# kelaendi/mused

Hardware: AMD Instinct MI355X
Metric: stream rows/sec, d=1024 l=128 window=10k synthetic (SWFD + kNN similarity + eigenstep + labels) (higher is better)
Workload: dtype f64; 1 GPU; synthetic d=1024 l=128 window=10000 k=50 (BASELINE config 2); stream=blob, W=10000, d=1024, l=128, k=50, modalities=1, swfd_levels=14, rccl_ranks=1, lanes_per_gpu=20, padded_window_slots=2

## Files before the change

### include/mused_hip.h

```cpp
#ifndef MUSED_HIP_H
#define MUSED_HIP_H

#ifdef __cplusplus
extern "C" {
#endif

#define MUSED_OK 0
#define MUSED_ERR_ARG -1
#define MUSED_ERR_HIP -2
#define MUSED_ERR_STATE -3
#define MUSED_ERR_UNSUPPORTED -4

#define MUSED_F32 0
#define MUSED_F64 1
#define MUSED_I64 2
#define MUSED_BITS 3

#define MUSED_METRIC_L2 0
#define MUSED_METRIC_COSINE 1

const char* mused_last_error(void);
int mused_version(void);
int mused_memcpy_d2d(void* dst, const void* src, long bytes, void* stream);

// ... 117 lines not shown
int mused_spmm_binary_path(int n, int r, long ldq, long ldy, int q_align, int y_align);
int mused_spmm_force_path(int path);
int mused_lu_permute_l(double* Y, int n, int r, long ld, int* ws_int, double* ws_f64, void* stream);
int mused_lu_mode(void);
int mused_lu_path(int n, int r);
int mused_qr_economic(double* Y, int n, int r, long ldy, double* Q, long ldq, double* ws_f64, void* stream);
int mused_syevj_batched(const double* G, int n, int batch, int sweeps, double* evals, double* V, void* stream);
int mused_gemm_f64(int a_kc, int b_kc, const double* A, long lda, const double* B, long ldb, double* C, long ldc,
                   int M, int N, int K, double alpha, void* stream);
int mused_gemm_f64_batched(int a_kc, int b_kc, const double* A, long lda, long strideA, const double* B, long ldb,
                           long strideB, double* C, long ldc, long strideC, int M, int N, int K, int batch,
                           double alpha, void* stream);
int mused_gemm_f64_batched_rep(int a_kc, int b_kc, const double* A, long lda, long strideA, const double* B, long ldb,
                               long strideB, double* C, long ldc, long strideC, int M, int N, int K, int batch,
                               double alpha, const int* rep, void* stream);
int mused_gemm_f64_splitk(int a_kc, int b_kc, const double* A, long lda, const double* B, long ldb, double* partial,
                          double* C, int M, int N, int K, int kchunk, int nsplit, void* stream);
int mused_gemm_f64_batched_splitk(int a_kc, int b_kc, const double* A, long lda, long strideA, const double* B, long ldb,
                                  long strideB, double* partial, double* C, int M, int N, int K, int batch, int kchunk,
                                  int nsplit, const int* rep, void* stream);
int mused_kmeans_assign_rows(int d, int k);

long mused_kmeans_ws_bytes(int n, int d, int k);
int mused_kmeans_lloyd(const double* X, long ld, int n, int d, int k, const double* mean, double* centers, double tol,
                       int max_iter, int* labels_out, int* info_out, void* ws, long ws_bytes, void* stream);
long mused_kmeans_wide_ws_bytes(int n, int d, int k);
int mused_kmeans_lloyd_wide(const double* X, long ld, int n, int d, int k, const double* mean, double* centers, double tol,
                            int max_iter, int* labels_out, int* info_out, void* ws, long ws_bytes, void* stream);
int mused_kmeans_wide_tiles(int d, int k, int* out);

// ... 83 lines not shown
```

### mused_amd/_lib.py

```python
from __future__ import annotations

import ctypes as C
import os

F32, F64, I64, BITS = 0, 1, 2, 3
METRIC_L2, METRIC_COSINE = 0, 1

_HERE = os.path.dirname(os.path.abspath(__file__))
LIB_PATH = os.path.join(_HERE, "lib", "libmused_hip.so")

_lib = None


class MusedError(RuntimeError):
    pass


_vp, _i, _l, _d = C.c_void_p, C.c_int, C.c_long, C.c_double

_PROTOS = {
    "mused_last_error": (C.c_char_p, []),
    "mused_version": (_i, []),
    "mused_memcpy_d2d": (_i, [_vp, _vp, _l, _vp]),
    "mused_row_sq_norms": (_i, [_vp, _i, _l, _i, _l, _vp, _vp]),
# ... 45 lines not shown
    "mused_rsvd_status": (_i, [_vp, C.POINTER(_i), C.POINTER(_i), _vp]),
    "mused_rsvd_cholqr": (_i, [_vp, _vp, _i, _i, _vp, _vp, _vp, _vp, _vp]),
    "mused_rsvd_select": (_i, [_vp, _vp, _vp, _vp, _i, _i, _i, _vp, _vp, _vp]),
    "mused_spmm_binary": (_i, [_vp, _vp, _i, _vp, _l, _i, _vp, _l, _vp]),
    "mused_spmm_valued": (_i, [_vp, _vp, _vp, _i, _vp, _l, _i, _vp, _l, _vp]),
    "mused_spmm_binary_path": (_i, [_i, _i, _l, _l, _i, _i]),
    "mused_spmm_force_path": (_i, [_i]),
    "mused_lu_permute_l": (_i, [_vp, _i, _i, _l, _vp, _vp, _vp]),
    "mused_lu_mode": (_i, []),
    "mused_lu_path": (_i, [_i, _i]),
    "mused_qr_economic": (_i, [_vp, _i, _i, _l, _vp, _l, _vp, _vp]),
    "mused_syevj_batched": (_i, [_vp, _i, _i, _i, _vp, _vp, _vp]),
    "mused_gemm_f64": (_i, [_i, _i, _vp, _l, _vp, _l, _vp, _l, _i, _i, _i, _d, _vp]),
    "mused_gemm_f64_batched": (_i, [_i, _i, _vp, _l, _l, _vp, _l, _l, _vp, _l, _l, _i, _i, _i, _i, _d, _vp]),
    "mused_gemm_f64_batched_rep": (_i, [_i, _i, _vp, _l, _l, _vp, _l, _l, _vp, _l, _l, _i, _i, _i, _i, _d, _vp, _vp]),
    "mused_gemm_f64_splitk": (_i, [_i, _i, _vp, _l, _vp, _l, _vp, _vp, _i, _i, _i, _i, _i, _vp]),
    "mused_gemm_f64_batched_splitk": (_i, [_i, _i, _vp, _l, _l, _vp, _l, _l, _vp, _vp, _i, _i, _i, _i, _i, _i, _vp, _vp]),
    "mused_kmeans_ws_bytes": (_l, [_i, _i, _i]),
    "mused_kmeans_lloyd": (_i, [_vp, _l, _i, _i, _i, _vp, _vp, _d, _i, _vp, C.POINTER(_i), _vp, _l, _vp]),
    "mused_kmeans_assign_rows": (_i, [_i, _i]),
    "mused_kmeans_wide_ws_bytes": (_l, [_i, _i, _i]),
    "mused_kmeans_lloyd_wide": (_i, [_vp, _l, _i, _i, _i, _vp, _vp, _d, _i, _vp, C.POINTER(_i), _vp, _l, _vp]),
    "mused_kmeans_wide_tiles": (_i, [_i, _i, C.POINTER(_i)]),
    "mused_kmeans_moments": (_i, [_vp, _l, _i, _i, _vp, _vp, _vp]),
    "mused_kmeans_seed_ws_bytes": (_l, [_i, _i, _i]),
    "mused_kmeans_seed": (_i, [_vp, _l, _i, _i, _i, _vp, _i, _vp, _i, _vp, _vp, _vp, _vp, _l, _vp]),
    "mused_mbkm_ws_bytes": (_l, [_i, _i, _i]),
    "mused_mbkm_step": (_i, [_vp, _l, _i, _i, _i, _vp, _vp, _vp, _vp, _l, _vp]),
    "mused_mbkm_reassign": (_i, [_vp, _l, _i, _i, _i, _vp, _vp, _i, _vp, _vp, _vp, _vp]),
    "mused_kmeans_assign": (_i, [_vp, _l, _i, _i, _i, _vp, _vp, _vp, _l, _vp]),
# ... 72 lines not shown
```

### mused_amd/csrc/gemm_f64.h

```cpp
#pragma once
#include <cstdlib>
#include <mutex>
#include <type_traits>
#include "common.h"

namespace mused {

typedef double v4f64 __attribute__((ext_vector_type(4)));

constexpr int GEMM_BM = 128;
constexpr int GEMM_BN = 128;
constexpr int GEMM_BK = 16;
constexpr int GEMM_LD = 144;
constexpr int GEMM_THREADS = 256;
constexpr int GEMM_LDS_BYTES = 2  * 2  * GEMM_BK * GEMM_LD * 8;

struct GemmArgs {
  const void* A;
  const void* B;
  long lda, ldb;
  long strideA, strideB;
  int M, N, K;
  int kchunk;
  int splitk;
  int bsplit;
  int tiles_m, tiles_n;
  const int* rep;
  const int* list;
  const int* kact;
  int sym;
};

template <typename TIn, bool VEC>
__device__ __forceinline__ void stage_load_kc(const TIn* __restrict__ src, long ld, int r0, int nrows, int k0,
                                              int kend, TIn (&r)[8]) {
  const int m = threadIdx.x & 127;
  const int kh = threadIdx.x >> 7;
  const int row = r0 + m;
  const int k = k0 + kh * 8;
  if (row < nrows) {
    const TIn* p = src + (long)row * ld + k;
    if (VEC && k + 8 <= kend) {
      if (sizeof(TIn) == 4) {
        const float4 a = *reinterpret_cast<const float4*>(p);
        const float4 b = *reinterpret_cast<const float4*>(p + 4);
// ... 82 lines not shown
      const double2 v = q[j];
      r[2 * j] = v.x;
      r[2 * j + 1] = v.y;
    }
  }
}
template <typename TIn>
__device__ __forceinline__ void stage_load_kc_full(const TIn* __restrict__ src, long ld, int r0, int k0, TIn (&r)[8]) {
  stage_load8(src + (long)(r0 + (threadIdx.x & 127)) * ld + k0 + (threadIdx.x >> 7) * 8, r);
}
template <typename TIn>
__device__ __forceinline__ void stage_load_mc_full(const TIn* __restrict__ src, long ld, int c0, int k0, TIn (&r)[8]) {
  stage_load8(src + (long)(k0 + (threadIdx.x >> 4)) * ld + c0 + (threadIdx.x & 15) * 8, r);
}

__device__ __forceinline__ int xcd_remap(int pid, int nwg) {
  const int q = nwg >> 3, r = nwg & 7, xcd = pid & 7;
  const int base = (xcd < r) ? xcd * (q + 1) : r * (q + 1) + (xcd - r) * q;
  return base + (pid >> 3);
}

template <typename TA, typename TB, bool A_KC, bool B_KC, bool VEC>
__device__ __forceinline__ void gemm_tile_mainloop(const GemmArgs& g, const TA* __restrict__ A, const TB* __restrict__ B,
                                                   int m0, int n0, int k_lo, int k_hi, double* smem,
                                                   v4f64 (&acc)[4][4]) {
  double* As = smem;
  double* Bs = smem + 2 * GEMM_BK * GEMM_LD;
  const int lane = threadIdx.x & 63;
  const int wave = threadIdx.x >> 6;
  const int wr = wave >> 1, wc = wave & 1;
  const int kq = lane >> 4, li = lane & 15;
#pragma unroll
  for (int i = 0; i < 4; ++i)
#pragma unroll
    for (int j = 0; j < 4; ++j) acc[i][j] = (v4f64){0.0, 0.0, 0.0, 0.0};

  TA ra[8];
  TB rb[8];
  const int nkt = (k_hi - k_lo + GEMM_BK - 1) / GEMM_BK;

  const bool full_mn = VEC && m0 + GEMM_BM <= g.M && n0 + GEMM_BN <= g.N;
  auto load_tile = [&](int kt) {
    const int k0 = k_lo + kt * GEMM_BK;
    if (full_mn && k0 + GEMM_BK <= k_hi) {
      if (A_KC) stage_load_kc_full<TA>(A, g.lda, m0, k0, ra); else stage_load_mc_full<TA>(A, g.lda, m0, k0, ra);
      if (B_KC) stage_load_kc_full<TB>(B, g.ldb, n0, k0, rb); else stage_load_mc_full<TB>(B, g.ldb, n0, k0, rb);
      return;
    }
    if (A_KC) stage_load_kc<TA, VEC>(A, g.lda, m0, g.M, k0, k_hi, ra);
    else      stage_load_mc<TA, VEC>(A, g.lda, m0, g.M, k0, k_hi, ra);
    if (B_KC) stage_load_kc<TB, VEC>(B, g.ldb, n0, g.N, k0, k_hi, rb);
    else      stage_load_mc<TB, VEC>(B, g.ldb, n0, g.N, k0, k_hi, rb);
  };
  auto store_tile = [&](int buf) {
    double* a = As + buf * GEMM_BK * GEMM_LD;
    double* b = Bs + buf * GEMM_BK * GEMM_LD;
    if (A_KC) stage_store_kc(a, ra); else stage_store_mc(a, ra);
    if (B_KC) stage_store_kc(b, rb); else stage_store_mc(b, rb);
  };

  if (nkt > 0) {
    load_tile(0);
    store_tile(0);
  }
  __syncthreads();

  int cur = 0;
  for (int kt = 0; kt < nkt; ++kt) {
    const bool more = (kt + 1 < nkt);
    if (more) load_tile(kt + 1);
    const double* a = As + cur * GEMM_BK * GEMM_LD + wr * 64 + li;
    const double* b = Bs + cur * GEMM_BK * GEMM_LD + wc * 64 + li;
// ... 281 lines not shown

struct EpiStore {
  double* C;
  long ldc;
  long strideC;
  double alpha;
  __device__ __forceinline__ void operator()(int z, int row, int col, double v) const {
    C[(long)z * strideC + (long)row * ldc + col] = alpha * v;
  }
  __device__ __forceinline__ double value(int, int, double v) const { return alpha * v; }
  __device__ __forceinline__ void put(int z, int row, int col, double val) const {
    C[(long)z * strideC + (long)row * ldc + col] = val;
  }
};

template <typename TA, typename TB, bool A_KC, bool B_KC, bool VEC, typename Epi>
int gemm_f64_prepare_t() {
  static std::once_flag once;
  static hipError_t err = hipSuccess;
  std::call_once(once, [] {
    auto k = gemm_f64_kernel<TA, TB, A_KC, B_KC, VEC, Epi>;
    err = hipFuncSetAttribute(reinterpret_cast<const void*>(k), hipFuncAttributeMaxDynamicSharedMemorySize,
                              GEMM_LDS_BYTES);
  });
  MUSED_CHECK_HIP(err);
  return MUSED_OK;
}

template <typename TA, typename TB, bool A_KC, bool B_KC, typename Epi>
int gemm_f64_launch_t(GemmArgs g, int batch, Epi epi, bool vec, hipStream_t stream) {
// ... 27 lines not shown
```

### mused_amd/csrc/gemm_f64.hip

```cpp
#include <stdarg.h>

#include "gemm_f64.h"
#include "internal.h"

namespace mused {

static thread_local char g_err[512] = "";

void set_error(const char* fmt, ...) {
  va_list ap;
  va_start(ap, fmt);
  vsnprintf(g_err, sizeof(g_err), fmt, ap);
  va_end(ap);
}

const char* last_error() { return g_err; }

int gemm_f64_prepare_all() {
  int rc = 0;
#define PREP(a, b, v) rc |= gemm_f64_prepare_t<double, double, a, b, v, EpiStore>()
  PREP(true, true, true); PREP(true, true, false); PREP(true, false, true); PREP(true, false, false);
  PREP(false, true, true); PREP(false, true, false); PREP(false, false, true); PREP(false, false, false);
#undef PREP
  return rc ? MUSED_ERR_HIP : MUSED_OK;
}

int gemm_f64(bool a_kc, bool b_kc, const double* A, long lda, long strideA, const double* B, long ldb,
             long strideB, double* C, long ldc, long strideC, int M, int N, int K, int batch, double alpha,
             hipStream_t stream, const int* rep, const int* list, const int* kact) {
  GemmArgs g;
  memset(&g, 0, sizeof(g));
  g.A = A; g.B = B; g.lda = lda; g.ldb = ldb; g.strideA = strideA; g.strideB = strideB;
  g.M = M; g.N = N; g.K = K; g.splitk = 0; g.kchunk = 0;
  g.rep = rep; g.list = list; g.kact = kact;
  g.sym = (A == B && a_kc == b_kc && lda == ldb && strideA == strideB && M == N) ? 1 : 0;
  EpiStore epi{C, ldc, strideC, alpha};
  const bool vec = vec_ok<double>(A, lda, strideA) && vec_ok<double>(B, ldb, strideB);
  if (a_kc && b_kc) return gemm_f64_launch_t<double, double, true, true>(g, batch, epi, vec, stream);
  if (a_kc && !b_kc) return gemm_f64_launch_t<double, double, true, false>(g, batch, epi, vec, stream);
  if (!a_kc && b_kc) return gemm_f64_launch_t<double, double, false, true>(g, batch, epi, vec, stream);
  return gemm_f64_launch_t<double, double, false, false>(g, batch, epi, vec, stream);
}

int gemm_f64_splitk(bool a_kc, bool b_kc, const double* A, long lda, const double* B, long ldb, double* partial,
                    int M, int N, int K, int kchunk, int nsplit, hipStream_t stream) {
  MUSED_REQUIRE(kchunk > 0 && kchunk % GEMM_BK == 0 && nsplit >= 1 && (long)kchunk * nsplit >= K,
                "gemm_f64_splitk: bad kchunk %d x %d for K=%d", kchunk, nsplit, K);
  GemmArgs g;
  memset(&g, 0, sizeof(g));
  g.A = A; g.B = B; g.lda = lda; g.ldb = ldb;
  g.M = M; g.N = N; g.K = K; g.splitk = 1; g.kchunk = kchunk;
  EpiStore epi{partial, (long)N, (long)M * N, 1.0};
// ... 84 lines not shown

int mused_gemm_f64_batched(int a_kc, int b_kc, const double* A, long lda, long strideA, const double* B, long ldb,
                           long strideB, double* C, long ldc, long strideC, int M, int N, int K, int batch,
                           double alpha, void* stream) {
  return mused::gemm_f64(a_kc != 0, b_kc != 0, A, lda, strideA, B, ldb, strideB, C, ldc, strideC, M, N, K, batch,
                         alpha, (hipStream_t)stream);
}

int mused_gemm_f64_batched_rep(int a_kc, int b_kc, const double* A, long lda, long strideA, const double* B, long ldb,
                               long strideB, double* C, long ldc, long strideC, int M, int N, int K, int batch,
                               double alpha, const int* rep, void* stream) {
  return mused::gemm_f64(a_kc != 0, b_kc != 0, A, lda, strideA, B, ldb, strideB, C, ldc, strideC, M, N, K, batch,
                         alpha, (hipStream_t)stream, rep);
}

int mused_debug_gemm_f64_batched_active(int a_kc, int b_kc, const double* A, long lda, long strideA, const double* B, long ldb,
                                        long strideB, double* C, long ldc, long strideC, int M, int N, int K, int batch,
                                        double alpha, const int* list, const int* kact, void* stream) {
  return mused::gemm_f64(a_kc != 0, b_kc != 0, A, lda, strideA, B, ldb, strideB, C, ldc, strideC, M, N, K, batch,
                         alpha, (hipStream_t)stream, nullptr, list, kact);
}

int mused_gemm_f64_splitk(int a_kc, int b_kc, const double* A, long lda, const double* B, long ldb, double* partial,
                          double* C, int M, int N, int K, int kchunk, int nsplit, void* stream) {
  MUSED_REQUIRE(A && B && partial && C && M >= 0 && N >= 0 && K >= 0, "mused_gemm_f64_splitk: bad arguments");
  int rc = mused::gemm_f64_splitk(a_kc != 0, b_kc != 0, A, lda, B, ldb, partial, M, N, K, kchunk, nsplit,
                                  (hipStream_t)stream);
  if (rc != MUSED_OK || M == 0 || N == 0) return rc;
  return mused::gemm_splitk_reduce(partial, nsplit, (long)M * N, C, (hipStream_t)stream);
}
// ... 14 lines not shown
```

### mused_amd/csrc/internal.h

```cpp
#pragma once
#include "common.h"

#include <mutex>

namespace mused {

int select_from_records(const double* rec, int n, int kind, int k, int* out_idx, unsigned long long* out_mask,
                        int mask_words, hipStream_t stream);
int select_from_tag_sets(const int* rowptr, const int* tags, const int* postptr, const int* postrow, int n, int k,
                         int* out_idx, unsigned long long* out_mask, int mask_words, hipStream_t stream);
int select_max_fused_rows(bool tag_sets);
int select_window_records(const double* rec, const int* vrank, int s, int e, int kind, int k, unsigned long long* out_mask,
                          int mask_words, hipStream_t stream);
int select_window_tag_sets(const int* rowptr, const int* tags, const int* postptr, const int* postrow, const int* vrank, int s,
                           int e, int k, unsigned long long* out_mask, int mask_words, hipStream_t stream);

std::recursive_mutex& capture_mutex();
using CaptureLock = std::lock_guard<std::recursive_mutex>;


int gemm_f64(bool a_kc, bool b_kc, const double* A, long lda, long strideA, const double* B, long ldb,
             long strideB, double* C, long ldc, long strideC, int M, int N, int K, int batch, double alpha,
             hipStream_t stream, const int* rep = nullptr, const int* list = nullptr, const int* kact = nullptr);

int gemm_f64_batched_splitk(bool a_kc, bool b_kc, const double* A, long lda, long strideA, const double* B, long ldb, long strideB,
                            double* partial, int M, int N, int K, int batch, int kchunk, int nsplit, hipStream_t stream,
                            const int* rep = nullptr, const int* list = nullptr);
int gemm_batched_splitk_reduce(const double* partial, int nsplit, long count, double* out, int batch, const int* rep,
                               hipStream_t stream, const int* list = nullptr);
int gemm_f64_prepare_all();

int gemm_f64_splitk(bool a_kc, bool b_kc, const double* A, long lda, const double* B, long ldb, double* partial,
                    int M, int N, int K, int kchunk, int nsplit, hipStream_t stream);
int gemm_splitk_reduce(const double* partial, int nsplit, long count, double* out, hipStream_t stream);

int lu_permute_l(double* Y, int n, int r, long ld, int* pivstep, double* prow, long ws_f64_len, hipStream_t st);
int qr_economic(double* Y, int n, int r, long ldy, double* Q, long ldq, double* tau, double* wpart, hipStream_t st,
                const int* run_if = nullptr);
// ... 70 lines not shown
```

### mused_amd/csrc/swfd.hip

```cpp
#include <vector>

#include "internal.h"

namespace mused {

struct Swfd {
  int N, d, ell, L, S, cap, n2, n4, n3;
  int lanes;
  double R;
  long i;
  int pend;
  long restart_mark;
  int skip_dead;
  bool twin;
  int sweeps;
  double* buf;
  bool tail_dirty;
  bool settle;
  int* used;
  double* queue;
  long long* qt;
  int* meta;
  int* rep;
  int* list;
  int* offs;
  int oround;
  int* kact;
  long long* ostat;
  long long* dropped;
  double* theta;
  double *T, *Wc;
  int gram_split;
  double* gpart;
  int* plan;
  int* keep_src;
  long long* now_dev;
  int* status;
  int* status_host;
  EigPlan* eig;
  double *stack, *Wq, *Bout, *sig_out, *qinfo;
  int* qsel;
  EigPlan* eigq;
  EigPlan* eigq3;
  int pre_chunk;
  double *pre_in, *pre_out, *pre_gram;
  EigPlan* eigp;
// ... 142 lines not shown
  __syncthreads();
  if (t == 0) list[0] = s_hist[16];
  if (t == 0) ostat[0] += 1;
  if (t == 1) ostat[1] += s_hist[16];
  if (t < 16) ostat[2 + t] += s_hist[t];
}

__global__ __launch_bounds__(1024) void swfd_decide_kernel(const double* __restrict__ evals,
                                                          const double* __restrict__ U, int ldu, int n2,
                                                          int ell, int cap,
                                                          int N, const long long* __restrict__ now_p,
                                                          const double* __restrict__ theta, int* __restrict__ meta,
                                                          long long* __restrict__ qt, long long* __restrict__ dropped,
                                                          int* __restrict__ plan, int* __restrict__ keep_src,
                                                          double* __restrict__ Wc, const int* __restrict__ rep,
                                                          int* __restrict__ used, int pend) {
  __shared__ double lam[1024];
  __shared__ int order[1024];
  __shared__ double scale[512];
  const int s = blockIdx.x, t = threadIdx.x;
  const long long now = *now_p;
  const int sr = rep ? rep[s] : s;
  if (sr < 0) return;
  const double* ev = evals + (long)sr * ldu;
  const double* Us = U + (long)sr * ldu * ldu;
  if (t < n2) lam[t] = ev[t];
  __syncthreads();
  if (t < n2) {
    const double mine = lam[t];
    int rank = 0;
    for (int j = 0; j < n2; ++j) {
// ... 74 lines not shown
      pos = (head1 + cnt1 + dpos) % cap;
      q[pos] = now;
    }
    plan[(s * ell + t) * 2 + 0] = kind;
    plan[(s * ell + t) * 2 + 1] = pos;
  }
  if (t == 0) {
    if (used) used[s] = min(n2, meta[s * 4 + 0] + pend);
    meta[s * 4 + 0] = nk;
    meta[s * 4 + 1] = (head1 + nevict) % cap;
    meta[s * 4 + 2] = cnt1 + nd - nevict;
    meta[s * 4 + 3] += nnear;
  }
  __syncthreads();
  if (sr != s) return;
  double* W = Wc + (long)s * ell * n2;
  for (int e = t; e < ell * n2; e += 1024) {
    const int i = e / n2, a = e - i * n2;
    const double sc = scale[i];
    W[e] = (sc != 0.0) ? sc * Us[(long)order[i] * ldu + a] : 0.0;
  }
}

__global__ void swfd_scatter_kernel(const double* __restrict__ T, const int* __restrict__ plan,
                                    const int* __restrict__ keep_src, const int* __restrict__ meta,
                                    double* __restrict__ buf, double* __restrict__ queue, int n2, int ell, int cap,
                                    int d, const int* __restrict__ rep) {
  const int rho = blockIdx.x, s = blockIdx.y;
  if (rep && rep[s] < 0) return;
  const double* Ts = T + (long)(rep ? rep[s] : s) * ell * d;
// ... 54 lines not shown
    hipLaunchKernelGGL(swfd_set_now_kernel, dim3(1), dim3(1), 0, st, h->now_dev, (long long)h->i);
  if (h->gram_split > 1) {
    const int kchunk = ((d + h->gram_split - 1) / h->gram_split + 15) / 16 * 16;
    if ((rc = gemm_f64_batched_splitk(true, true, h->buf, d, (long)n2 * d, h->buf, d, (long)n2 * d, h->gpart, n2, n2, d, S, kchunk,
                                      h->gram_split, st, h->rep, h->list)))
      return rc;
    if ((rc = gemm_batched_splitk_reduce(h->gpart, h->gram_split, (long)n2 * n2, eig_plan_input(h->eig), S, h->rep, st, h->list)))
      return rc;
  } else if ((rc = gemm_f64(true, true, h->buf, d, (long)n2 * d, h->buf, d, (long)n2 * d, eig_plan_input(h->eig), n2,
                            (long)n2 * n2, n2, n2, d, S, 1.0, st, h->rep, h->list)))
    return rc;
  if ((rc = eig_plan_run_inplace(h->eig, nullptr, nullptr, st, true))) return rc;
  const EigColumns e = eig_plan_columns(h->eig);
  hipLaunchKernelGGL(swfd_decide_kernel, dim3(S), dim3(1024), 0, st, e.lam, e.cols, e.ld, n2, ell, h->cap, h->N, h->now_dev,
                     h->theta, h->meta, h->qt, h->dropped, h->plan, h->keep_src, h->Wc, h->rep, h->settle ? h->used : nullptr,
                     h->pend);
  if ((rc = gemm_f64(true, false, h->Wc, n2, (long)ell * n2, h->buf, d, (long)n2 * d, h->T, d, (long)ell * d, ell, d,
                     n2, S, 1.0, st, h->rep, h->list, h->kact)))
    return rc;
  if (h->settle) {
    hipLaunchKernelGGL(swfd_settle_kernel<Src>, dim3(n2, S), dim3(256), 0, st, h->T, h->plan, h->keep_src, h->meta, h->used,
                       h->tail_dirty ? 1 : 0, h->buf, h->queue, n2, ell, h->cap, d, h->rep, next, ldx, lane_stride, 2 * h->L,
                       nxt);
    h->tail_dirty = false;
  } else {
    hipLaunchKernelGGL(swfd_scatter_kernel, dim3(n2, S), dim3(256), 0, st, h->T, h->plan, h->keep_src, h->meta, h->buf,
                       h->queue, n2, ell, h->cap, d, h->rep);
  }
  MUSED_LAUNCH_CHECK();
  h->pend = 0;
  return MUSED_OK;
}

static int swfd_restart(Swfd* h, hipStream_t st) {
// ... 159 lines not shown
                                  double* __restrict__ stack) {
  const int rho = blockIdx.x, lane = blockIdx.y;
  const int* qsel = qsel_all + (long)lane * (4 + cap);
  const int ns = qsel[1], nk = qsel[2], sk = qsel[3];
  const double* src = nullptr;
  if (rho < ns) src = queue + ((long)sk * cap + qsel[4 + rho]) * d;
  else if (rho < ns + nk + pend) src = buf + ((long)sk * n2 + (rho - ns)) * d;
  double* dst = stack + ((long)lane * n4 + rho) * d;
  for (int c = threadIdx.x; c < d; c += blockDim.x) dst[c] = src ? src[c] : 0.0;
}

__global__ __launch_bounds__(1024) void swfd_decide_query_kernel(const double* __restrict__ evals_all,
                                                                const double* __restrict__ U_all, int ldu, int n4, int ell,
                                                                int cap, const int* __restrict__ qsel_all,
                                                                double* __restrict__ Wq_all,
                                                                double* __restrict__ qinfo_all) {
  __shared__ double lam[1024];
  __shared__ int order[1024];
  __shared__ double scale[512];
  const int t = threadIdx.x, lane = blockIdx.x;
  const double* evals = evals_all + (long)lane * ldu;
  const double* U = U_all + (long)lane * ldu * ldu;
  const int* qsel = qsel_all + (long)lane * (4 + cap);
  double* Wq = Wq_all + (long)lane * ell * n4;
  double* qinfo = qinfo_all + (long)lane * 2;
  if (t < n4) lam[t] = evals[t];
  __syncthreads();
  if (t < n4) {
    const double mine = lam[t];
    int rank = 0;
    for (int j = 0; j < n4; ++j) {
      const double o = lam[j];
      rank += (o > mine) || (o == mine && j < t);
    }
    order[rank] = t;
  }
  __syncthreads();
  const double l0 = lam[order[0]];
  const double delta = lam[order[ell - 1]] > 0.0 ? lam[order[ell - 1]] : 0.0;
  const double tol = 1e-10 * (l0 > 0.0 ? l0 : 0.0);
  if (t < ell) {
    const double l = lam[order[t]];
    double s2 = l - delta;
    s2 = s2 > 0.0 ? s2 : 0.0;
    scale[t] = (s2 > tol) ? sqrt(s2 / l) / l : 0.0;
  }
  if (t == 0) {
    qinfo[0] = (double)qsel[0];
    qinfo[1] = delta;
  }
  __syncthreads();
  for (int e = t; e < ell * n4; e += 1024) {
    const int i = e / n4, a = e - i * n4;
    const double sc = scale[i];
    Wq[e] = (sc != 0.0) ? sc * U[(long)order[i] * ldu + a] : 0.0;
  }
}

__global__ __launch_bounds__(256) void swfd_finish_rows_kernel(double* __restrict__ B, int d, double* __restrict__ sig) {
  __shared__ double sv[4];
  __shared__ int si[4];
  __shared__ double ss[4];
  __shared__ double s_sign;
  const long rowid = (long)blockIdx.y * gridDim.x + blockIdx.x;
  double* row = B + rowid * d;
  double best = -1.0, sq = 0.0;
// ... 27 lines not shown
static int swfd_query(Swfd* h, double* outB, double* outSigma, double* outInfo, hipStream_t st) {
  const bool small = (h->pend == 0) && h->eigq3;
  EigPlan* const eq = small ? h->eigq3 : h->eigq;
  const int n4 = small ? h->n3 : h->n4, d = h->d, ell = h->ell, B = h->lanes;
  int rc;
  hipLaunchKernelGGL(swfd_select_kernel, dim3(B), dim3(64), 0, st, h->meta, h->qt, h->dropped, h->L, h->cap, h->N,
                     (long long)h->i, h->qsel);
  hipLaunchKernelGGL(swfd_stack_kernel, dim3(n4, B), dim3(256), 0, st, h->qsel, h->buf, h->queue, h->n2, n4, h->cap, d,
                     h->pend, h->stack);
  if ((rc = gemm_f64(true, true, h->stack, d, (long)n4 * d, h->stack, d, (long)n4 * d, eig_plan_input(eq), n4,
                     (long)n4 * n4, n4, n4, d, B, 1.0, st)))
    return rc;
  if ((rc = eig_plan_run_inplace(eq, nullptr, nullptr, st, true))) return rc;
  const EigColumns e = eig_plan_columns(eq);
  hipLaunchKernelGGL(swfd_decide_query_kernel, dim3(B), dim3(1024), 0, st, e.lam, e.cols, e.ld, n4, ell, h->cap, h->qsel, h->Wq,
                     h->qinfo);
  if ((rc = gemm_f64(true, false, h->Wq, n4, (long)ell * n4, h->stack, d, (long)n4 * d, h->Bout, d, (long)ell * d, ell,
                     d, n4, B, 1.0, st)))
    return rc;
  hipLaunchKernelGGL(swfd_finish_rows_kernel, dim3(ell, B), dim3(256), 0, st, h->Bout, d, h->sig_out);
  MUSED_LAUNCH_CHECK();
  MUSED_CHECK_HIP(hipMemcpyAsync(outB, h->Bout, sizeof(double) * (size_t)B * ell * d, hipMemcpyDeviceToDevice, st));
  if (outSigma)
    MUSED_CHECK_HIP(hipMemcpyAsync(outSigma, h->sig_out, sizeof(double) * (size_t)B * ell, hipMemcpyDeviceToDevice, st));
  if (outInfo) MUSED_CHECK_HIP(hipMemcpyAsync(outInfo, h->qinfo, sizeof(double) * 2 * B, hipMemcpyDeviceToDevice, st));
  return MUSED_OK;
}

static size_t swfd_half_bytes(const Swfd* h) {
  const size_t L = h->L;
  return L * ((size_t)h->n2 * h->d * 8 + (size_t)h->cap * h->d * 8 + (size_t)h->cap * 8 + 4 * 4 + 8);
}

}
// ... 60 lines not shown
      if (!off("MUSED_SWFD_ORDERS")) ZALLOC(h->offs, 4 * S);
      const char* orr = getenv("MUSED_SWFD_ORDERS");
      const int rv = orr ? atoi(orr) : 0;
      h->oround = (rv == 1 || rv == 16 || rv == 32) ? rv : SWFD_OFFS_ROUND;
      if (!off("MUSED_SWFD_KACT")) ZALLOC(h->kact, 4 * S);
    }
    const char* sd = getenv("MUSED_SWFD_SKIP_DEAD");
    h->skip_dead = (sd && sd[0] == '0') ? 0 : 1;
    h->settle = !off("MUSED_SWFD_SETTLE");
    if (h->settle) ZALLOC(h->used, 4 * S);
  }
  ZALLOC(h->dropped, 8 * S);
  ZALLOC(h->status, 4);
  MUSED_CHECK_HIP(hipHostMalloc((void**)&h->status_host, sizeof(int), hipHostMallocDefault));
  ALLOC(h->theta, 8 * S);
  ALLOC(h->T, 8 * S * l * dd); ALLOC(h->Wc, 8 * S * l * n2);
  ALLOC(h->plan, 4 * S * l * 2); ALLOC(h->keep_src, 4 * S * l); ALLOC(h->now_dev, 8);
  {
    const char* gs = getenv("MUSED_SWFD_GRAM_SPLIT");
    h->gram_split = gs ? atoi(gs) : (d >= 8192 ? 8 : 1);
    if (h->gram_split < 1 || h->gram_split > 16) h->gram_split = 1;
    if (h->gram_split > 1) ALLOC(h->gpart, 8 * S * (size_t)h->gram_split * n2 * n2);
  }
  const size_t Bn = lanes;
  ALLOC(h->stack, 8 * Bn * n4 * dd);
  ALLOC(h->Wq, 8 * Bn * l * n4); ALLOC(h->Bout, 8 * Bn * l * dd); ALLOC(h->sig_out, 8 * Bn * l);
  ALLOC(h->qinfo, 8 * 2 * Bn); ALLOC(h->qsel, 4 * Bn * (4 + cap));
#undef ZALLOC
#undef ALLOC
  std::vector<double> th(S);
  for (int lane = 0; lane < lanes; ++lane)
    for (int kind = 0; kind < 2; ++kind)
      for (int j = 0; j < h->L; ++j) th[sk_index(h, lane, j, kind)] = ldexp((double)h->N / ell, j);
  MUSED_CHECK_HIP(hipMemcpy(h->theta, th.data(), 8 * S, hipMemcpyHostToDevice));
  int rc;
  if ((rc = gemm_f64_prepare_all())) return rc;
  if ((rc = eig_plan_create(h->n2, h->S, h->sweeps, true, &h->eig, h->rep, EIG_PLAN_TOP_HALF, h->status, 0, h->list, h->offs)))
    return rc;
  if ((rc = eig_plan_create(h->n4, lanes, h->sweeps + 2, true, &h->eigq, nullptr, EIG_PLAN_TOP_FD, h->status, ell))) return rc;
  if (h->n3 < h->n4 &&
      (rc = eig_plan_create(h->n3, lanes, h->sweeps + 2, true, &h->eigq3, nullptr, EIG_PLAN_TOP_FD, h->status, ell)))
// ... 17 lines not shown
    }
  }
  return MUSED_OK;
}

int mused_swfd_destroy(void* handle) {
  Swfd* h = (Swfd*)handle;
  if (!h) return MUSED_OK;
  CaptureLock resource_guard(capture_mutex());
  eig_plan_destroy(h->eig);
  eig_plan_destroy(h->eigq);
  if (h->eigq3) eig_plan_destroy(h->eigq3);
  if (h->eigp) eig_plan_destroy(h->eigp);
  void* bufs[] = {h->buf, h->queue, h->qt, h->meta, h->dropped, h->theta, h->T, h->Wc, h->plan,
                  h->keep_src, h->now_dev, h->stack, h->Wq, h->Bout, h->sig_out, h->qinfo, h->qsel,
                  h->rep, h->pre_in, h->pre_out, h->pre_gram, h->status, h->gpart, h->list, h->offs, h->kact, h->ostat, h->used};
  for (void* b : bufs) (void)hipFree(b);
  if (h->status_host) (void)hipHostFree(h->status_host);
  delete h;
  return MUSED_OK;
}

int mused_swfd_levels(void* handle) { return handle ? ((Swfd*)handle)->L : -1; }

int mused_swfd_profile(void* handle, int on) {
  Swfd* h = (Swfd*)handle;
  MUSED_REQUIRE(h, "mused_swfd_profile: null handle");
  return eig_plan_profile(h->eig, on != 0);
}

int mused_swfd_profile_read(void* handle, double* total_ms, long* launches, double* bytes_per_launch) {
// ... 177 lines not shown
```

Before: 651,400 rows/s.

## Gather scaled eigenvector rows inside the GEMM instead of materializing Wc/Wq

The decide kernels no longer write a dense scaled-eigenvector weight matrix (Wc, Wq). They emit only a per-output-row source index and scale. A new gathered-row GEMM kernel reads eigenvector rows directly from the eigensolver output and applies the scale while staging them into LDS. This removes the writes and re-reads of the ell×n2 weight matrices, but adds per-thread row indirection and a new GEMM specialization. The old path stays available through MUSED_SWFD_WC=1.

```diff
diff --git a/include/mused_hip.h b/include/mused_hip.h
--- a/include/mused_hip.h
+++ b/include/mused_hip.h
@@ -155,6 +155,10 @@
 int mused_gemm_f64_batched_rep(int a_kc, int b_kc, const double* A, long lda, long strideA, const double* B, long ldb,
                                long strideB, double* C, long ldc, long strideC, int M, int N, int K, int batch,
                                double alpha, const int* rep, void* stream);
+int mused_gemm_f64_batched_rows(int a_kc, int b_kc, const double* A, long lda, long strideA, const double* B, long ldb,
+                                long strideB, double* C, long ldc, long strideC, int M, int N, int K, int batch,
+                                double alpha, const int* arow, const double* ascale, const int* rep_or_null,
+                                const int* kact_or_null, void* stream);
 int mused_gemm_f64_splitk(int a_kc, int b_kc, const double* A, long lda, const double* B, long ldb, double* partial,
                           double* C, int M, int N, int K, int kchunk, int nsplit, void* stream);
 int mused_gemm_f64_batched_splitk(int a_kc, int b_kc, const double* A, long lda, long strideA, const double* B, long ldb,
diff --git a/mused_amd/_lib.py b/mused_amd/_lib.py
--- a/mused_amd/_lib.py
+++ b/mused_amd/_lib.py
@@ -83,6 +83,8 @@
     "mused_gemm_f64": (_i, [_i, _i, _vp, _l, _vp, _l, _vp, _l, _i, _i, _i, _d, _vp]),
     "mused_gemm_f64_batched": (_i, [_i, _i, _vp, _l, _l, _vp, _l, _l, _vp, _l, _l, _i, _i, _i, _i, _d, _vp]),
     "mused_gemm_f64_batched_rep": (_i, [_i, _i, _vp, _l, _l, _vp, _l, _l, _vp, _l, _l, _i, _i, _i, _i, _d, _vp, _vp]),
+    "mused_gemm_f64_batched_rows": (_i, [_i, _i, _vp, _l, _l, _vp, _l, _l, _vp, _l, _l, _i, _i, _i, _i, _d, _vp, _vp, _vp,
+                                         _vp, _vp]),
     "mused_gemm_f64_splitk": (_i, [_i, _i, _vp, _l, _vp, _l, _vp, _vp, _i, _i, _i, _i, _i, _vp]),
     "mused_gemm_f64_batched_splitk": (_i, [_i, _i, _vp, _l, _l, _vp, _l, _l, _vp, _vp, _i, _i, _i, _i, _i, _i, _vp, _vp]),
     "mused_kmeans_ws_bytes": (_l, [_i, _i, _i]),
diff --git a/mused_amd/csrc/gemm_f64.h b/mused_amd/csrc/gemm_f64.h
--- a/mused_amd/csrc/gemm_f64.h
+++ b/mused_amd/csrc/gemm_f64.h
@@ -29,6 +29,9 @@
   const int* list;
   const int* kact;
   int sym;
+  const int* arow;
+  const double* ascale;
+  long stride_rows;
 };
 
 template <typename TIn, bool VEC>
@@ -141,16 +144,36 @@
   stage_load8(src + (long)(k0 + (threadIdx.x >> 4)) * ld + c0 + (threadIdx.x & 15) * 8, r);
 }
 
+template <bool VEC>
+__device__ __forceinline__ void stage_load_row(const double* __restrict__ prow, int k0, int kend, double (&r)[8]) {
+  const int k = k0 + (threadIdx.x >> 7) * 8;
+  const double* p = prow + k;
+  if (VEC && k + 8 <= kend) {
+    stage_load8(p, r);
+  } else {
+#pragma unroll
+    for (int j = 0; j < 8; ++j) r[j] = (k + j < kend) ? p[j] : 0.0;
+  }
+}
+__device__ __forceinline__ void stage_store_kc_scaled(double* __restrict__ lds, const double (&r)[8], double s) {
+  const int m = threadIdx.x & 127;
+  const int kh = threadIdx.x >> 7;
+#pragma unroll
+  for (int j = 0; j < 8; ++j) lds[(kh * 8 + j) * GEMM_LD + m] = (s != 0.0) ? s * r[j] : 0.0;
+}
+
 __device__ __forceinline__ int xcd_remap(int pid, int nwg) {
   const int q = nwg >> 3, r = nwg & 7, xcd = pid & 7;
   const int base = (xcd < r) ? xcd * (q + 1) : r * (q + 1) + (xcd - r) * q;
   return base + (pid >> 3);
 }
 
-template <typename TA, typename TB, bool A_KC, bool B_KC, bool VEC>
+template <typename TA, typename TB, bool A_KC, bool B_KC, bool VEC, bool GATHER = false>
 __device__ __forceinline__ void gemm_tile_mainloop(const GemmArgs& g, const TA* __restrict__ A, const TB* __restrict__ B,
                                                    int m0, int n0, int k_lo, int k_hi, double* smem,
-                                                   v4f64 (&acc)[4][4]) {
+                                                   v4f64 (&acc)[4][4], const double* __restrict__ prow = nullptr,
+                                                   double ascl = 0.0) {
+  static_assert(!GATHER || (A_KC && std::is_same<TA, double>::value), "gathered A: K-contiguous fp64 only");
   double* As = smem;
   double* Bs = smem + 2 * GEMM_BK * GEMM_LD;
   const int lane = threadIdx.x & 63;
@@ -170,11 +193,13 @@
   auto load_tile = [&](int kt) {
     const int k0 = k_lo + kt * GEMM_BK;
     if (full_mn && k0 + GEMM_BK <= k_hi) {
-      if (A_KC) stage_load_kc_full<TA>(A, g.lda, m0, k0, ra); else stage_load_mc_full<TA>(A, g.lda, m0, k0, ra);
+      if constexpr (GATHER) stage_load8(prow + k0 + (threadIdx.x >> 7) * 8, ra);
+      else if (A_KC) stage_load_kc_full<TA>(A, g.lda, m0, k0, ra); else stage_load_mc_full<TA>(A, g.lda, m0, k0, ra);
       if (B_KC) stage_load_kc_full<TB>(B, g.ldb, n0, k0, rb); else stage_load_mc_full<TB>(B, g.ldb, n0, k0, rb);
       return;
     }
-    if (A_KC) stage_load_kc<TA, VEC>(A, g.lda, m0, g.M, k0, k_hi, ra);
+    if constexpr (GATHER) stage_load_row<VEC>(prow, k0, k_hi, ra);
+    else if (A_KC) stage_load_kc<TA, VEC>(A, g.lda, m0, g.M, k0, k_hi, ra);
     else      stage_load_mc<TA, VEC>(A, g.lda, m0, g.M, k0, k_hi, ra);
     if (B_KC) stage_load_kc<TB, VEC>(B, g.ldb, n0, g.N, k0, k_hi, rb);
     else      stage_load_mc<TB, VEC>(B, g.ldb, n0, g.N, k0, k_hi, rb);
@@ -182,7 +207,8 @@
   auto store_tile = [&](int buf) {
     double* a = As + buf * GEMM_BK * GEMM_LD;
     double* b = Bs + buf * GEMM_BK * GEMM_LD;
-    if (A_KC) stage_store_kc(a, ra); else stage_store_mc(a, ra);
+    if constexpr (GATHER) stage_store_kc_scaled(a, ra, ascl);
+    else if (A_KC) stage_store_kc(a, ra); else stage_store_mc(a, ra);
     if (B_KC) stage_store_kc(b, rb); else stage_store_mc(b, rb);
   };
 
@@ -494,6 +520,68 @@
   }
 };
 
+template <bool VEC>
+__global__ __launch_bounds__(GEMM_THREADS, 2) void gemm_f64_rows_kernel(GemmArgs g, EpiStore epi) {
+  extern __shared__ __attribute__((aligned(16))) double smem[];
+
+  int zb = blockIdx.z;
+  if (g.list) {
+    if (zb >= g.list[0]) return;
+    zb = g.list[1 + zb];
+  } else if (g.rep && g.rep[zb] != zb) return;
+  const int nwg = g.tiles_m * g.tiles_n;
+  const int wg = xcd_remap(blockIdx.x, nwg);
+  constexpr int GROUP_M = 8;
+  const int per_group = GROUP_M * g.tiles_n;
+  const int first_m = (wg / per_group) * GROUP_M;
+  const int group_size = min(g.tiles_m - first_m, GROUP_M);
+  const int m0 = (first_m + (wg % group_size)) * GEMM_BM, n0 = ((wg % per_group) / group_size) * GEMM_BN;
+  const int k_hi = g.kact ? min(g.K, g.kact[zb]) : g.K;
+  const double* A = reinterpret_cast<const double*>(g.A) + (long)zb * g.strideA;
+  const double* B = reinterpret_cast<const double*>(g.B) + (long)zb * g.strideB;
+
+  const int mrow = m0 + (threadIdx.x & 127);
+  const long mi = (long)zb * g.stride_rows + min(mrow, g.M - 1);
+  const double s_in = g.ascale[mi];
+  const int r_in = g.arow[mi];
+  const bool live = mrow < g.M && s_in != 0.0;
+  const double ascl = live ? s_in : 0.0;
+  const double* prow = A + (long)(live ? r_in : 0) * g.lda;
+
+  const int lane = threadIdx.x & 63;
+  const int wave = threadIdx.x >> 6;
+  const int wr = wave >> 1, wc = wave & 1;
+  const int kq = lane >> 4, li = lane & 15;
+
+  v4f64 acc[4][4];
+  gemm_tile_mainloop<double, double, true, false, VEC, true>(g, A, B, m0, n0, 0, k_hi, smem, acc, prow, ascl);
+
+#pragma unroll
+  for (int i = 0; i < 4; ++i) {
+#pragma unroll
+    for (int j = 0; j < 4; ++j) {
+      const int col = n0 + wc * 64 + j * 16 + li;
+#pragma unroll
+      for (int r = 0; r < 4; ++r) {
+        const int row = m0 + wr * 64 + i * 16 + kq + 4 * r;
+        if (row < g.M && col < g.N) epi(zb, row, col, acc[i][j][r]);
+      }
+    }
+  }
+}
+
+template <bool VEC>
+int gemm_f64_rows_prepare_t() {
+  static std::once_flag once;
+  static hipError_t err = hipSuccess;
+  std::call_once(once, [] {
+    err = hipFuncSetAttribute(reinterpret_cast<const void*>(gemm_f64_rows_kernel<VEC>),
+                              hipFuncAttributeMaxDynamicSharedMemorySize, GEMM_LDS_BYTES);
+  });
+  MUSED_CHECK_HIP(err);
+  return MUSED_OK;
+}
+
 template <typename TA, typename TB, bool A_KC, bool B_KC, bool VEC, typename Epi>
 int gemm_f64_prepare_t() {
   static std::once_flag once;
diff --git a/mused_amd/csrc/gemm_f64.hip b/mused_amd/csrc/gemm_f64.hip
--- a/mused_amd/csrc/gemm_f64.hip
+++ b/mused_amd/csrc/gemm_f64.hip
@@ -22,12 +22,32 @@
   PREP(true, true, true); PREP(true, true, false); PREP(true, false, true); PREP(true, false, false);
   PREP(false, true, true); PREP(false, true, false); PREP(false, false, true); PREP(false, false, false);
 #undef PREP
+  rc |= gemm_f64_rows_prepare_t<true>();
+  rc |= gemm_f64_rows_prepare_t<false>();
   return rc ? MUSED_ERR_HIP : MUSED_OK;
+}
+
+static int gemm_f64_rows_launch(GemmArgs g, int batch, EpiStore epi, bool vec, hipStream_t stream) {
+  g.tiles_m = cdiv(g.M, GEMM_BM);
+  g.tiles_n = cdiv(g.N, GEMM_BN);
+  if (g.M <= 0 || g.N <= 0 || batch <= 0) return MUSED_OK;
+  dim3 grid(g.tiles_m * g.tiles_n, 1, batch);
+  int rc;
+  if (vec) {
+    if ((rc = gemm_f64_rows_prepare_t<true>())) return rc;
+    hipLaunchKernelGGL(gemm_f64_rows_kernel<true>, grid, dim3(GEMM_THREADS), GEMM_LDS_BYTES, stream, g, epi);
+  } else {
+    if ((rc = gemm_f64_rows_prepare_t<false>())) return rc;
+    hipLaunchKernelGGL(gemm_f64_rows_kernel<false>, grid, dim3(GEMM_THREADS), GEMM_LDS_BYTES, stream, g, epi);
+  }
+  MUSED_LAUNCH_CHECK();
+  return MUSED_OK;
 }
 
 int gemm_f64(bool a_kc, bool b_kc, const double* A, long lda, long strideA, const double* B, long ldb,
              long strideB, double* C, long ldc, long strideC, int M, int N, int K, int batch, double alpha,
-             hipStream_t stream, const int* rep, const int* list, const int* kact) {
+             hipStream_t stream, const int* rep, const int* list, const int* kact, const int* arow, const double* ascale,
+             long stride_rows) {
   GemmArgs g;
   memset(&g, 0, sizeof(g));
   g.A = A; g.B = B; g.lda = lda; g.ldb = ldb; g.strideA = strideA; g.strideB = strideB;
@@ -36,6 +56,13 @@
   g.sym = (A == B && a_kc == b_kc && lda == ldb && strideA == strideB && M == N) ? 1 : 0;
   EpiStore epi{C, ldc, strideC, alpha};
   const bool vec = vec_ok<double>(A, lda, strideA) && vec_ok<double>(B, ldb, strideB);
+  if (arow || ascale) {
+    MUSED_REQUIRE(arow && ascale, "gemm_f64: a row map and row scales come together");
+    MUSED_REQUIRE(a_kc && !b_kc && !g.sym, "gemm_f64: gathered rows need a K-contiguous A, a [K][N] B and no symmetric launch");
+    MUSED_REQUIRE(stride_rows >= 0, "gemm_f64: negative row map stride %ld", stride_rows);
+    g.arow = arow; g.ascale = ascale; g.stride_rows = stride_rows;
+    return gemm_f64_rows_launch(g, batch, epi, vec, stream);
+  }
   if (a_kc && b_kc) return gemm_f64_launch_t<double, double, true, true>(g, batch, epi, vec, stream);
   if (a_kc && !b_kc) return gemm_f64_launch_t<double, double, true, false>(g, batch, epi, vec, stream);
   if (!a_kc && b_kc) return gemm_f64_launch_t<double, double, false, true>(g, batch, epi, vec, stream);
@@ -150,6 +177,15 @@
                          alpha, (hipStream_t)stream, rep);
 }
 
+int mused_gemm_f64_batched_rows(int a_kc, int b_kc, const double* A, long lda, long strideA, const double* B, long ldb,
+                                long strideB, double* C, long ldc, long strideC, int M, int N, int K, int batch,
+                                double alpha, const int* arow, const double* ascale, const int* rep_or_null,
+                                const int* kact_or_null, void* stream) {
+  MUSED_REQUIRE(arow && ascale, "mused_gemm_f64_batched_rows: null row map or scales");
+  return mused::gemm_f64(a_kc != 0, b_kc != 0, A, lda, strideA, B, ldb, strideB, C, ldc, strideC, M, N, K, batch,
+                         alpha, (hipStream_t)stream, rep_or_null, nullptr, kact_or_null, arow, ascale, (long)M);
+}
+
 int mused_debug_gemm_f64_batched_active(int a_kc, int b_kc, const double* A, long lda, long strideA, const double* B, long ldb,
                                         long strideB, double* C, long ldc, long strideC, int M, int N, int K, int batch,
                                         double alpha, const int* list, const int* kact, void* stream) {
diff --git a/mused_amd/csrc/internal.h b/mused_amd/csrc/internal.h
--- a/mused_amd/csrc/internal.h
+++ b/mused_amd/csrc/internal.h
@@ -21,7 +21,8 @@
 
 int gemm_f64(bool a_kc, bool b_kc, const double* A, long lda, long strideA, const double* B, long ldb,
              long strideB, double* C, long ldc, long strideC, int M, int N, int K, int batch, double alpha,
-             hipStream_t stream, const int* rep = nullptr, const int* list = nullptr, const int* kact = nullptr);
+             hipStream_t stream, const int* rep = nullptr, const int* list = nullptr, const int* kact = nullptr,
+             const int* arow = nullptr, const double* ascale = nullptr, long stride_rows = 0);
 
 int gemm_f64_batched_splitk(bool a_kc, bool b_kc, const double* A, long lda, long strideA, const double* B, long ldb, long strideB,
                             double* partial, int M, int N, int K, int batch, int kchunk, int nsplit, hipStream_t stream,
diff --git a/mused_amd/csrc/swfd.hip b/mused_amd/csrc/swfd.hip
--- a/mused_amd/csrc/swfd.hip
+++ b/mused_amd/csrc/swfd.hip
@@ -30,6 +30,8 @@
   long long* dropped;
   double* theta;
   double *T, *Wc;
+  int* wrow;
+  double* wscale;
   int gram_split;
   double* gpart;
   int* plan;
@@ -202,7 +204,8 @@
                                                           long long* __restrict__ qt, long long* __restrict__ dropped,
                                                           int* __restrict__ plan, int* __restrict__ keep_src,
                                                           double* __restrict__ Wc, const int* __restrict__ rep,
-                                                          int* __restrict__ used, int pend) {
+                                                          int* __restrict__ used, int pend, int* __restrict__ wrow,
+                                                          double* __restrict__ wscale) {
   __shared__ double lam[1024];
   __shared__ int order[1024];
   __shared__ double scale[512];
@@ -307,6 +310,13 @@
   }
   __syncthreads();
   if (sr != s) return;
+  if (!Wc) {
+    if (t < ell) {
+      wrow[s * ell + t] = order[t];
+      wscale[s * ell + t] = scale[t];
+    }
+    return;
+  }
   double* W = Wc + (long)s * ell * n2;
   for (int e = t; e < ell * n2; e += 1024) {
     const int i = e / n2, a = e - i * n2;
@@ -391,10 +401,12 @@
   const EigColumns e = eig_plan_columns(h->eig);
   hipLaunchKernelGGL(swfd_decide_kernel, dim3(S), dim3(1024), 0, st, e.lam, e.cols, e.ld, n2, ell, h->cap, h->N, h->now_dev,
                      h->theta, h->meta, h->qt, h->dropped, h->plan, h->keep_src, h->Wc, h->rep, h->settle ? h->used : nullptr,
-                     h->pend);
-  if ((rc = gemm_f64(true, false, h->Wc, n2, (long)ell * n2, h->buf, d, (long)n2 * d, h->T, d, (long)ell * d, ell, d,
-                     n2, S, 1.0, st, h->rep, h->list, h->kact)))
-    return rc;
+                     h->pend, h->wrow, h->wscale);
+  rc = h->Wc ? gemm_f64(true, false, h->Wc, n2, (long)ell * n2, h->buf, d, (long)n2 * d, h->T, d, (long)ell * d, ell, d, n2, S,
+                        1.0, st, h->rep, h->list, h->kact)
+             : gemm_f64(true, false, e.cols, e.ld, (long)e.ld * e.ld, h->buf, d, (long)n2 * d, h->T, d, (long)ell * d, ell, d,
+                        n2, S, 1.0, st, h->rep, h->list, h->kact, h->wrow, h->wscale, ell);
+  if (rc) return rc;
   if (h->settle) {
     hipLaunchKernelGGL(swfd_settle_kernel<Src>, dim3(n2, S), dim3(256), 0, st, h->T, h->plan, h->keep_src, h->meta, h->used,
                        h->tail_dirty ? 1 : 0, h->buf, h->queue, n2, ell, h->cap, d, h->rep, next, ldx, lane_stride, 2 * h->L,
@@ -584,7 +596,8 @@
                                                                 const double* __restrict__ U_all, int ldu, int n4, int ell,
                                                                 int cap, const int* __restrict__ qsel_all,
                                                                 double* __restrict__ Wq_all,
-                                                                double* __restrict__ qinfo_all) {
+                                                                double* __restrict__ qinfo_all, int* __restrict__ wrow,
+                                                                double* __restrict__ wscale) {
   __shared__ double lam[1024];
   __shared__ int order[1024];
   __shared__ double scale[512];
@@ -592,7 +605,7 @@
   const double* evals = evals_all + (long)lane * ldu;
   const double* U = U_all + (long)lane * ldu * ldu;
   const int* qsel = qsel_all + (long)lane * (4 + cap);
-  double* Wq = Wq_all + (long)lane * ell * n4;
+  double* Wq = Wq_all ? Wq_all + (long)lane * ell * n4 : nullptr;
   double* qinfo = qinfo_all + (long)lane * 2;
   if (t < n4) lam[t] = evals[t];
   __syncthreads();
@@ -620,6 +633,13 @@
     qinfo[1] = delta;
   }
   __syncthreads();
+  if (!Wq) {
+    if (t < ell) {
+      wrow[lane * ell + t] = order[t];
+      wscale[lane * ell + t] = scale[t];
+    }
+    return;
+  }
   for (int e = t; e < ell * n4; e += 1024) {
     const int i = e / n4, a = e - i * n4;
     const double sc = scale[i];
@@ -677,10 +697,12 @@
   if ((rc = eig_plan_run_inplace(eq, nullptr, nullptr, st, true))) return rc;
   const EigColumns e = eig_plan_columns(eq);
   hipLaunchKernelGGL(swfd_decide_query_kernel, dim3(B), dim3(1024), 0, st, e.lam, e.cols, e.ld, n4, ell, h->cap, h->qsel, h->Wq,
-                     h->qinfo);
-  if ((rc = gemm_f64(true, false, h->Wq, n4, (long)ell * n4, h->stack, d, (long)n4 * d, h->Bout, d, (long)ell * d, ell,
-                     d, n4, B, 1.0, st)))
-    return rc;
+                     h->qinfo, h->wrow, h->wscale);
+  rc = h->Wq ? gemm_f64(true, false, h->Wq, n4, (long)ell * n4, h->stack, d, (long)n4 * d, h->Bout, d, (long)ell * d, ell, d,
+                        n4, B, 1.0, st)
+             : gemm_f64(true, false, e.cols, e.ld, (long)e.ld * e.ld, h->stack, d, (long)n4 * d, h->Bout, d, (long)ell * d, ell,
+                        d, n4, B, 1.0, st, nullptr, nullptr, nullptr, h->wrow, h->wscale, ell);
+  if (rc) return rc;
   hipLaunchKernelGGL(swfd_finish_rows_kernel, dim3(ell, B), dim3(256), 0, st, h->Bout, d, h->sig_out);
   MUSED_LAUNCH_CHECK();
   MUSED_CHECK_HIP(hipMemcpyAsync(outB, h->Bout, sizeof(double) * (size_t)B * ell * d, hipMemcpyDeviceToDevice, st));
@@ -771,7 +793,15 @@
   ZALLOC(h->status, 4);
   MUSED_CHECK_HIP(hipHostMalloc((void**)&h->status_host, sizeof(int), hipHostMallocDefault));
   ALLOC(h->theta, 8 * S);
-  ALLOC(h->T, 8 * S * l * dd); ALLOC(h->Wc, 8 * S * l * n2);
+  ALLOC(h->T, 8 * S * l * dd);
+  const char* wcs = getenv("MUSED_SWFD_WC");
+  const bool wc_path = wcs && wcs[0] == '1';
+  if (wc_path) {
+    ALLOC(h->Wc, 8 * S * l * n2);
+  } else {
+    ALLOC(h->wrow, 4 * S * l);
+    ALLOC(h->wscale, 8 * S * l);
+  }
   ALLOC(h->plan, 4 * S * l * 2); ALLOC(h->keep_src, 4 * S * l); ALLOC(h->now_dev, 8);
   {
     const char* gs = getenv("MUSED_SWFD_GRAM_SPLIT");
@@ -781,7 +811,8 @@
   }
   const size_t Bn = lanes;
   ALLOC(h->stack, 8 * Bn * n4 * dd);
-  ALLOC(h->Wq, 8 * Bn * l * n4); ALLOC(h->Bout, 8 * Bn * l * dd); ALLOC(h->sig_out, 8 * Bn * l);
+  if (wc_path) ALLOC(h->Wq, 8 * Bn * l * n4);
+  ALLOC(h->Bout, 8 * Bn * l * dd); ALLOC(h->sig_out, 8 * Bn * l);
   ALLOC(h->qinfo, 8 * 2 * Bn); ALLOC(h->qsel, 4 * Bn * (4 + cap));
 #undef ZALLOC
 #undef ALLOC
@@ -829,7 +860,8 @@
   if (h->eigp) eig_plan_destroy(h->eigp);
   void* bufs[] = {h->buf, h->queue, h->qt, h->meta, h->dropped, h->theta, h->T, h->Wc, h->plan,
                   h->keep_src, h->now_dev, h->stack, h->Wq, h->Bout, h->sig_out, h->qinfo, h->qsel,
-                  h->rep, h->pre_in, h->pre_out, h->pre_gram, h->status, h->gpart, h->list, h->offs, h->kact, h->ostat, h->used};
+                  h->rep, h->pre_in, h->pre_out, h->pre_gram, h->status, h->gpart, h->list, h->offs, h->kact, h->ostat, h->used,
+                  h->wrow, h->wscale};
   for (void* b : bufs) (void)hipFree(b);
   if (h->status_host) (void)hipHostFree(h->status_host);
   delete h;
```

Measured after the change: 657,700 rows/s (median of 6 runs). No clear change (+1.0%).
